# meiqua/6DPose

Measured on AMD Instinct MI355X. Metric: templates*Mpixels matched/sec on 640x480 RGB-D, higher is better.
Workload: dtype u8

## Files before the change

6dpose_amd/csrc/match_bits.hip:

```cpp
#include "match_planes.h"
#include <algorithm>
#include <type_traits>

namespace lm {

static __device__ __forceinline__ uint32_t pack4(uint32_t d) {
    const uint32_t t = ((d | (d >> 1)) & 0x01010101u) | ((d >> 1) & 0x02020202u);
    return (t * 0x01041040u) >> 24;
}
static __device__ __forceinline__ uint32_t pack16(const uint4& v) { return pack4(v.x) | (pack4(v.y) << 8) | (pack4(v.z) << 16) | (pack4(v.w) << 24); }

__global__ void __launch_bounds__(256)
k_pack_bits(BitsBatch B, uint32_t sm_off0, uint32_t records, int NS, int Hd) {
    const uint32_t i = blockIdx.x * 256u + threadIdx.x;
    if (i >= records) return;
    uint4 a, b;
    const size_t at = strip_cells(B.strips[blockIdx.y], sm_off0, i, NS, Hd, a, b);
    uint2 r;
    r.x = pack16(a);
    r.y = pack16(b);
    *reinterpret_cast<uint2*>(B.bits[blockIdx.y] + at) = r;
}

template <int kHi, int kWaves, int kA>
__global__ void __launch_bounds__(256) __attribute__((amdgpu_waves_per_eu(kWaves, kWaves)))
k_local_bits(FrameBatch fb, BitsBatch B, FrameGeom g, const TemplEntry* __restrict__ entries, const uint32_t* __restrict__ feat_word,
             const int32_t* __restrict__ work_pyramids, uint32_t cand_cap, float threshold, uint32_t cap, uint32_t dedupe_cap_slots) {
    constexpr int kN = 4 + kHi;
    constexpr int kS = kN + 3;
    __shared__ unsigned long long s_acc[kMaxBatch][2];
    __shared__ uint32_t s_cnt[kMaxBatch];
    const int lane = threadIdx.x & 63, grp = lane >> 3, j = lane & 7;
    const int nb = fb.nb;
    const LocalShare share = local_share(nb);
    local_prologue(fb, s_cnt, s_acc, cand_cap, dedupe_cap_slots);
    if (B.top_clear_units)
        for (int f = 0; f < nb; ++f)
            for (uint32_t i = blockIdx.x * blockDim.x + threadIdx.x; i < B.top_clear_units; i += gridDim.x * blockDim.x)
                reinterpret_cast<uint4*>(B.top_clear[f])[i] = make_uint4(0u, 0u, 0u, 0u);
    const int src0 = (lane & ~7) << 2;
    const uint32_t rowoff = 16u * (uint32_t)j;
    for (int fr = share.f_lo; fr < share.f_hi; ++fr) {
        const FrameSlot& F = fb.f[fr];
        const BufRsrc bits = make_rsrc(B.bits[fr]);
        const uint32_t nc = s_cnt[fr], ngroups = (nc + 7u) >> 3;
        for (uint32_t gi = share.w_first; gi < ngroups; gi += share.w_step) {
            const uint32_t ci = gi * 8u + (uint32_t)grp;
            const bool valid = ci < nc;
            Candidate cd{0, 0, 0.f, 0};
            if (valid) cd = F.cands[ci];
            const int work = cd.work;
            const int pyr = work_pyramids[work];
            int mx = cd.x, my = cd.y;
            float sim = cd.score;
            bool alive = valid, leave = false;
            uint32_t evals = 0, bytes = 0;
            for (int l = g.levels - 2; l >= 0; --l) {
                const LevelGeom& lv = g.lv[l];
                const TemplEntry e = entries[(size_t)pyr * g.levels + l];
                const LocalWindow win = local_window(lv, e, mx, my, alive, leave);
                const int nfp = win.nfp, nmax = win.nmax;
                const uint32_t* fw = feat_word + e.feat_start;
                uint32_t cA[kN], cB[kN];
#pragma unroll
                for (int k = 0; k < kN; ++k) { cA[k] = 0; cB[k] = 0; }
                uint32_t offx = 0, offy = 0, sx = 0, sy = 0;
                auto batch = [&](int half, uint32_t& eA, uint32_t& eB) {
                    uint4 v[8];
                    uint32_t sh[8];
#pragma unroll
                    for (int u = 0; u < 8; ++u) {
                        const int src = src0 + 4 * (4 * half + (u >> 1));
                        const uint32_t o = (uint32_t)__builtin_amdgcn_ds_bpermute(src, (int)((u & 1) ? offy : offx));
                        sh[u] = (uint32_t)__builtin_amdgcn_ds_bpermute(src, (int)((u & 1) ? sy : sx));
                        v[u] = ld_buf16(bits, o + rowoff, 0u);
                    }
                    uint32_t xa[8], xb[8];
#pragma unroll
                    for (int u = 0; u < 8; ++u) {
                        xa[u] = __builtin_amdgcn_alignbit(v[u].y, v[u].x, sh[u]);
                        xb[u] = __builtin_amdgcn_alignbit(v[u].w, v[u].z, sh[u]);
                    }
                    eA = add8(xa, cA[0], cA[1], cA[2]);
                    eB = add8(xb, cB[0], cB[1], cB[2]);
                };
                uint2 wn = local_fetch(fw, 0, j, nfp);
                for (int f0 = 0; f0 < nmax; f0 += 16) {
                    const uint2 wd = wn;
                    const bool on = f0 + 2 * j < nfp;
                    wn = local_fetch(fw, f0 + 16, j, nfp);
                    local_prep(wd.x, on, win.gxl, win.Kbase, win.HS8, win.zero_off, offx, sx);
                    local_prep(wd.y, on, win.gxl, win.Kbase, win.HS8, win.zero_off, offy, sy);
                    uint32_t e1A, e1B;
                    batch(0, e1A, e1B);
                    if (f0 + 8 < nmax) {
                        uint32_t e2A, e2B;
                        batch(1, e2A, e2B);
                        add_eights2<kN>(cA, e1A, e2A);
                        add_eights2<kN>(cB, e1B, e2B);
                    } else {
                        add_eights1<kN>(cA, e1A);
                        add_eights1<kN>(cB, e1B);
                    }
                }
                uint32_t S[kS];
                {
                    uint32_t n1[kN], n4[kN];
                    local_interleave<kN>(n1, n4, cA, cB);
                    weighted_sum<kA, kN>(S, n1, n4);
                }
                int raw, br, bc;
                local_argmax<kS>(S, j, raw, br, bc);
                local_update(win, lv.T, raw, br, bc, threshold, sim, mx, my, alive, evals, bytes);
            }
            if (valid && j == 0) local_store(F, ci, leave, cap, mx, my, sim, alive, work, s_acc[fr], evals, bytes);
        }
    }
    local_flush_stats(fb, s_acc);
}

void launch_pack_bits(const BitsBatch& B, int nb, const LevelGeom& lv, hipStream_t s) {
    const uint32_t records = (uint32_t)(2 * 8 * lv.T * lv.T) * (uint32_t)lv.NS * (uint32_t)lv.Hd;
    hipLaunchKernelGGL(k_pack_bits, dim3((records + 255) / 256, nb), dim3(256), 0, s, B, lv.sm_off[0], records, lv.NS, lv.Hd);
}
void launch_local_bits(const FrameBatch& fb, const BitsBatch& B, const FrameGeom& g, const BankDev& bank, uint32_t cand_cap, float threshold,
                       uint32_t cap, uint32_t dedupe_cap_slots, int grid_blocks, int max_features, int low_weight, hipStream_t s) {
    with_bits_instance<4, 4>(max_features, low_weight, [&](auto hi, auto waves, auto a) {
        hipLaunchKernelGGL((k_local_bits<hi(), waves(), a()>), dim3(grid_blocks), dim3(256), 0, s, fb, B, g, bank.entries, bank.feat_word, bank.work, cand_cap, threshold, cap,
                           dedupe_cap_slots);
    });
}

__global__ void __launch_bounds__(256)
k_pack_top(TopBits B, uint32_t byte0, uint32_t npairs) {
    const uint32_t i = blockIdx.x * 256u + threadIdx.x;
    if (i >= npairs) return;
    const uint8_t* src = B.lm[blockIdx.y] + byte0 + (size_t)i * 32;
    const uint4 a = *reinterpret_cast<const uint4*>(src), b = *reinterpret_cast<const uint4*>(src + 16);
    *reinterpret_cast<uint2*>(B.bits[blockIdx.y] + (size_t)i * 8) = make_uint2(byte_bits32(a, b, 0) | byte_bits32(a, b, 1), byte_bits32(a, b, 2));
}

template <int kHi, int kWaves, int kA>
__global__ void __launch_bounds__(256) __attribute__((amdgpu_waves_per_eu(kWaves, kWaves)))
k_coarse_bits(FrameBatch fb, TopBits B, LevelGeom lv, int level, int levels, const TemplEntry* __restrict__ entries, const int32_t* __restrict__ feat_off,
              const int32_t* __restrict__ work_pyramids, int num_work, float threshold, uint32_t cap, uint32_t byte0) {
    constexpr int kN = 4 + kHi, kS = kN + 3;
    __shared__ uint32_t s_tot[4];
    __shared__ unsigned long long s_base;
    const FrameSlot& F = fb.f[blockIdx.y];
    const int lane = threadIdx.x & 63;
    const int wave = __builtin_amdgcn_readfirstlane((int)(threadIdx.x >> 6));
    const CoarseHead h = coarse_head((int)blockIdx.x * 4 + wave, num_work, entries, feat_off, work_pyramids, lv, level, levels, threshold);
    const bool live = h.live;
    const int nfp = h.nfp, npos = h.npos, limit = h.limit;
    const int32_t* fo = h.fo;
    const BufRsrc bits = make_rsrc(B.bits[blockIdx.y]);
    for (int P0 = 0; P0 < npos; P0 += 2048) {
        const int pos0 = P0 + 32 * lane;
        uint32_t c1[kN], c4[kN];
#pragma unroll
        for (int k = 0; k < kN; ++k) { c1[k] = 0; c4[k] = 0; }
        if (live && P0 < limit && nfp > 0 && pos0 < limit) {
            auto batch = [&](int f, uint32_t& e1, uint32_t& e4) {
                uint4 v[8];
                uint32_t sh[8];
#pragma unroll
                for (int u = 0; u < 8; ++u) {
                    const uint32_t ob = (uint32_t)fo[f + u] - byte0 + (uint32_t)P0;
                    sh[u] = ob & 31u;
                    v[u] = ld_buf16(bits, (uint32_t)lane * 8u, (ob >> 5) * 8u);
                }
                uint32_t x1[8], x4[8];
#pragma unroll
                for (int u = 0; u < 8; ++u) {
                    x1[u] = __builtin_amdgcn_alignbit(v[u].z, v[u].x, sh[u]);
                    x4[u] = __builtin_amdgcn_alignbit(v[u].w, v[u].y, sh[u]);
                }
                e1 = add8(x1, c1[0], c1[1], c1[2]);
                e4 = add8(x4, c4[0], c4[1], c4[2]);
            };
            for (int f = 0; f < nfp; f += 16) {
                uint32_t a1, a4;
                batch(f, a1, a4);
                if (f + 8 < nfp) {
                    uint32_t b1, b4;
                    batch(f + 8, b1, b4);
                    add_eights2<kN>(c1, a1, b1);
                    add_eights2<kN>(c4, a4, b4);
                } else {
                    add_eights1<kN>(c1, a1);
                    add_eights1<kN>(c4, a4);
                }
            }
        }
        uint32_t S[kS];
        weighted_sum<kA, kN>(S, c1, c4);
        uint32_t summed;
        uint32_t hit_mask = coarse_hit_mask<kS>(S, h.rmin, h.zero_passes, limit, npos, pos0, summed);
        if (!live) hit_mask = 0;
// ... 132 lines not shown
```

6dpose_amd/csrc/match_parts.hip:

```cpp
#include "match_planes.h"

namespace lm {

template <int kHi, int kWaves, int kA>
__global__ void __launch_bounds__(256) __attribute__((amdgpu_waves_per_eu(kWaves, kWaves)))
k_coarse_parts(FrameBatch fb, TopBits B, LevelGeom lv, int level, int levels, const TemplEntry* __restrict__ entries, const PartEntry* __restrict__ parts,
               const int32_t* __restrict__ part_off, const int32_t* __restrict__ work_pyramids, int num_work, float threshold, int min_parts, uint32_t cap, uint32_t byte0) {
    constexpr int kN = 4 + kHi, kS = kN + 3;
    __shared__ uint32_t s_tot[4];
    __shared__ unsigned long long s_base;
    const FrameSlot& F = fb.f[blockIdx.y];
    const int lane = threadIdx.x & 63;
    const int wave = __builtin_amdgcn_readfirstlane((int)(threadIdx.x >> 6));
    const CoarseHead h = coarse_head((int)blockIdx.x * 4 + wave, num_work, entries, part_off, work_pyramids, lv, level, levels, threshold);
    const bool live = h.live;
    const int npos = h.npos, limit = h.limit;
    const PartEntry* pe = parts + (size_t)work_pyramids[h.work] * levels + level;
    const BufRsrc bits = make_rsrc(B.bits[blockIdx.y]);
    for (int P0 = 0; P0 < npos; P0 += 2048) {
        const int pos0 = P0 + 32 * lane;
        const bool loads = live && P0 < limit && pos0 < limit;
        uint32_t S[kS];
#pragma unroll
        for (int k = 0; k < kS; ++k) S[k] = 0;
        uint32_t q0 = 0, q1 = 0, q2 = 0, summed = 0;
#pragma unroll 1
        for (int p = 0; p < 4; ++p) {
            const int np = pe->n[p], npp = pe->npad[p];
            const int32_t* fo = part_off + pe->start[p];
            uint32_t c1[kN], c4[kN];
#pragma unroll
            for (int k = 0; k < kN; ++k) { c1[k] = 0; c4[k] = 0; }
            if (loads) {
                auto batch = [&](int f, uint32_t& e1, uint32_t& e4) {
                    uint4 v[8];
                    uint32_t sh[8];
#pragma unroll
                    for (int u = 0; u < 8; ++u) {
                        const uint32_t ob = (uint32_t)fo[f + u] - byte0 + (uint32_t)P0;
                        sh[u] = ob & 31u;
                        v[u] = ld_buf16(bits, (uint32_t)lane * 8u, (ob >> 5) * 8u);
                    }
                    uint32_t x1[8], x4[8];
#pragma unroll
                    for (int u = 0; u < 8; ++u) {
                        x1[u] = __builtin_amdgcn_alignbit(v[u].z, v[u].x, sh[u]);
                        x4[u] = __builtin_amdgcn_alignbit(v[u].w, v[u].y, sh[u]);
                    }
                    e1 = add8(x1, c1[0], c1[1], c1[2]);
                    e4 = add8(x4, c4[0], c4[1], c4[2]);
                };
                for (int f = 0; f < npp; f += 16) {
                    uint32_t a1, a4;
                    batch(f, a1, a4);
                    if (f + 8 < npp) {
                        uint32_t b1, b4;
                        batch(f + 8, b1, b4);
                        add_eights2<kN>(c1, a1, b1);
                        add_eights2<kN>(c4, a4, b4);
                    } else {
                        add_eights1<kN>(c1, a1);
                        add_eights1<kN>(c4, a4);
                    }
                }
            }
            uint32_t Sp[kS];
            weighted_sum<kA, kN>(Sp, c1, c4);
            const int rmin = (pe->eligible >> p) & 1u ? coarse_rmin(threshold, np) : (1 << kS);
            count3_add(q0, q1, q2, coarse_hit_mask<kS>(Sp, rmin, false, limit, npos, pos0, summed));
            sliced_add<kS>(S, Sp);
        }
        uint32_t hit_mask = count3_ge(q0, q1, q2, min_parts);
        if (!live) hit_mask = 0;
        int total;
        const unsigned long long slot = coarse_reserve_slots(s_tot, s_base, F.counters, hit_mask, lane, wave, total);
        if (total > 0)
            coarse_emit<kS>(hit_mask, summed, S, slot, cap, pos0, h.Wd, h.T, h.offset, h.nf, h.work, F.cands);
    }
}

template <int kHi, int kWaves, int kA>
__global__ void __launch_bounds__(256) __attribute__((amdgpu_waves_per_eu(kWaves, kWaves)))
k_local_parts(FrameBatch fb, BitsBatch B, FrameGeom g, const TemplEntry* __restrict__ entries, const PartEntry* __restrict__ parts, const uint32_t* __restrict__ part_word,
              const int32_t* __restrict__ work_pyramids, uint32_t cand_cap, float threshold, int min_parts, uint32_t cap, uint32_t dedupe_cap_slots) {
    constexpr int kN = 4 + kHi;
    constexpr int kS = kN + 3;
    __shared__ unsigned long long s_acc[kMaxBatch][2];
    __shared__ uint32_t s_cnt[kMaxBatch];
    const int lane = threadIdx.x & 63, grp = lane >> 3, j = lane & 7;
    const int nb = fb.nb;
    const LocalShare share = local_share(nb);
    local_prologue(fb, s_cnt, s_acc, cand_cap, dedupe_cap_slots);
    if (B.top_clear_units)
        for (int f = 0; f < nb; ++f)
            for (uint32_t i = blockIdx.x * blockDim.x + threadIdx.x; i < B.top_clear_units; i += gridDim.x * blockDim.x)
                reinterpret_cast<uint4*>(B.top_clear[f])[i] = make_uint4(0u, 0u, 0u, 0u);
    const int src0 = (lane & ~7) << 2;
    const uint32_t rowoff = 16u * (uint32_t)j;
    for (int fr = share.f_lo; fr < share.f_hi; ++fr) {
        const FrameSlot& F = fb.f[fr];
        const BufRsrc bits = make_rsrc(B.bits[fr]);
        const uint32_t nc = s_cnt[fr], ngroups = (nc + 7u) >> 3;
        for (uint32_t gi = share.w_first; gi < ngroups; gi += share.w_step) {
            const uint32_t ci = gi * 8u + (uint32_t)grp;
            const bool valid = ci < nc;
            Candidate cd{0, 0, 0.f, 0};
            if (valid) cd = F.cands[ci];
            const int work = cd.work;
            const int pyr = work_pyramids[work];
            int mx = cd.x, my = cd.y;
            float sim = cd.score;
            bool alive = valid, leave = false;
            uint32_t evals = 0, bytes = 0;
            for (int l = g.levels - 2; l >= 0; --l) {
                const LevelGeom& lv = g.lv[l];
                const TemplEntry e = entries[(size_t)pyr * g.levels + l];
                const uint32_t ei = (uint32_t)(pyr * g.levels + l);
                const LocalWindow win = local_window(lv, e, mx, my, alive, leave);
                const int my_bound = (parts[ei].eligible >> (j & 3)) & 1u ? local_rmin(threshold, (int)parts[ei].n[j & 3]) : (1 << kS);
                uint32_t S[kS];
#pragma unroll
                for (int k = 0; k < kS; ++k) S[k] = 0;
                uint32_t q0 = 0, q1 = 0, q2 = 0;
#pragma unroll 1
                for (int p = 0; p < 4; ++p) {
                    const int nfp = win.run ? (int)parts[ei].npad[p] : 0;
                    int nmax = nfp;
#pragma unroll
                    for (int o = 32; o > 0; o >>= 1) { const int t = __shfl_xor(nmax, o, 64); nmax = t > nmax ? t : nmax; }
                    nmax = __builtin_amdgcn_readfirstlane(nmax);
                    const uint32_t* fw = part_word + parts[ei].start[p];
                    uint32_t cA[kN], cB[kN];
#pragma unroll
                    for (int k = 0; k < kN; ++k) { cA[k] = 0; cB[k] = 0; }
                    uint32_t offx = 0, offy = 0, sx = 0, sy = 0;
                    auto batch = [&](int half, uint32_t& eA, uint32_t& eB) {
                        uint4 v[8];
                        uint32_t sh[8];
#pragma unroll
                        for (int u = 0; u < 8; ++u) {
                            const int src = src0 + 4 * (4 * half + (u >> 1));
                            const uint32_t o = (uint32_t)__builtin_amdgcn_ds_bpermute(src, (int)((u & 1) ? offy : offx));
                            sh[u] = (uint32_t)__builtin_amdgcn_ds_bpermute(src, (int)((u & 1) ? sy : sx));
                            v[u] = ld_buf16(bits, o + rowoff, 0u);
                        }
                        uint32_t xa[8], xb[8];
#pragma unroll
                        for (int u = 0; u < 8; ++u) {
                            xa[u] = __builtin_amdgcn_alignbit(v[u].y, v[u].x, sh[u]);
                            xb[u] = __builtin_amdgcn_alignbit(v[u].w, v[u].z, sh[u]);
                        }
                        eA = add8(xa, cA[0], cA[1], cA[2]);
                        eB = add8(xb, cB[0], cB[1], cB[2]);
                    };
                    uint2 wn = local_fetch(fw, 0, j, nfp);
                    for (int f0 = 0; f0 < nmax; f0 += 16) {
                        const uint2 wd = wn;
                        const bool on = f0 + 2 * j < nfp;
                        wn = local_fetch(fw, f0 + 16, j, nfp);
                        local_prep(wd.x, on, win.gxl, win.Kbase, win.HS8, win.zero_off, offx, sx);
                        local_prep(wd.y, on, win.gxl, win.Kbase, win.HS8, win.zero_off, offy, sy);
                        uint32_t e1A, e1B;
                        batch(0, e1A, e1B);
                        if (f0 + 8 < nmax) {
                            uint32_t e2A, e2B;
                            batch(1, e2A, e2B);
                            add_eights2<kN>(cA, e1A, e2A);
                            add_eights2<kN>(cB, e1B, e2B);
                        } else {
                            add_eights1<kN>(cA, e1A);
                            add_eights1<kN>(cB, e1B);
                        }
                    }
                    uint32_t Sp[kS];
                    {
                        uint32_t n1[kN], n4[kN];
                        local_interleave<kN>(n1, n4, cA, cB);
                        weighted_sum<kA, kN>(Sp, n1, n4);
                    }
                    const int bound = __shfl(my_bound, (lane & ~7) + p, 64);
                    count3_add(q0, q1, q2, sliced_ge<kS>(Sp, bound));
                    sliced_add<kS>(S, Sp);
                }
                int raw, br, bc;
                local_argmax<kS>(S, j, raw, br, bc);
                const int at = raw > 0 ? 2 * bc + (br & 1) : 0;
                const int mine = (int)((q0 >> at) & 1u) + 2 * (int)((q1 >> at) & 1u) + 4 * (int)((q2 >> at) & 1u);
                const int passed = __shfl(mine, (lane & ~7) + (raw > 0 ? br >> 1 : 0), 64);
                local_update(win, lv.T, raw, br, bc, -__builtin_inff() , sim, mx, my, alive, evals, bytes);
                if (win.run && passed < min_parts) alive = false;
            }
            if (valid && j == 0) local_store(F, ci, leave, cap, mx, my, sim, alive, work, s_acc[fr], evals, bytes);
        }
    }
    local_flush_stats(fb, s_acc);
}

void launch_coarse_parts(const FrameBatch& fb, const TopBits& B, const FrameGeom& g, const BankDev& bank, const PartsDev& parts, int num_work, float threshold, uint32_t cap,
                         uint32_t byte0, int max_features, int low_weight, hipStream_t s) {
    if (num_work <= 0 || fb.nb <= 0) return;
    const int level = g.levels - 1;
    with_bits_instance<5, 4>(max_features, low_weight, [&](auto hi, auto waves, auto a) {
        hipLaunchKernelGGL((k_coarse_parts<hi(), waves(), a()>), dim3((num_work + 3) / 4, fb.nb), dim3(256), 0, s, fb, B, g.lv[level], level, g.levels, bank.entries, parts.table,
                           parts.feat_off, bank.work, num_work, threshold, parts.min_parts, cap, byte0);
    });
}
void launch_local_parts(const FrameBatch& fb, const BitsBatch& B, const FrameGeom& g, const BankDev& bank, const PartsDev& parts, uint32_t cand_cap, float threshold,
                        uint32_t cap, uint32_t dedupe_cap_slots, int grid_blocks, int max_features, int low_weight, hipStream_t s) {
    with_bits_instance<4, 3>(max_features, low_weight, [&](auto hi, auto waves, auto a) {
        hipLaunchKernelGGL((k_local_parts<hi(), waves(), a()>), dim3(grid_blocks), dim3(256), 0, s, fb, B, g, bank.entries, parts.table, parts.feat_word, bank.work, cand_cap, threshold,
                           parts.min_parts, cap, dedupe_cap_slots);
    });
}

}
```

6dpose_amd/csrc/match_planes.h:

```cpp
#pragma once
#include "match_device.h"
#include <type_traits>

namespace lm {


static __device__ __forceinline__ int coarse_rmin(float threshold, int nf) {
    int rmin = (int)(threshold * (float)(4 * nf) / 100.f);
    if (!(rmin >= 0)) rmin = 0;
    if (rmin > 4 * nf + 1) rmin = 4 * nf + 1;
    while (rmin > 0 && score_of(rmin, nf) > threshold) --rmin;
    while (rmin <= 4 * nf && !(score_of(rmin, nf) > threshold)) ++rmin;
    return rmin;
}

static __device__ __forceinline__ int local_rmin(float threshold, int nf) {
    int rmin = (int)(threshold * (float)(4 * nf) / 100.f);
    if (!(rmin >= 0)) rmin = 0;
    if (rmin > 4 * nf + 1) rmin = 4 * nf + 1;
    while (rmin > 0 && score_of(rmin - 1, nf) >= threshold) --rmin;
    while (rmin <= 4 * nf && !(score_of(rmin, nf) >= threshold)) ++rmin;
    return rmin;
}

struct CoarseHead {
    bool live;
    int work, nf, nfp;
    const int32_t* fo;
    int Wd, T, npos;
    int limit;
    int offset;
    int rmin;
    bool zero_passes;
};
static __device__ __forceinline__ CoarseHead coarse_head(int work_raw, int num_work, const TemplEntry* __restrict__ entries, const int32_t* __restrict__ feat_off,
                                                         const int32_t* __restrict__ work_pyramids, const LevelGeom& lv, int level, int levels, float threshold) {
    CoarseHead h;
    h.live = work_raw < num_work;
    h.work = h.live ? work_raw : num_work - 1;
    const int pyr = work_pyramids[h.work];
    const TemplEntry e = entries[(size_t)pyr * levels + level];
    h.nf = e.nf; h.nfp = e.nf_padded;
    h.fo = feat_off + e.feat_start;
    const int Hd = lv.Hd;
    h.Wd = lv.Wd; h.T = lv.T; h.npos = h.Wd * Hd;
    const int wf = (e.width - 1) / h.T + 1, hf = (e.height - 1) / h.T + 1;
    const int tp = (Hd - hf) * h.Wd + (h.Wd - wf) + 1;
    h.offset = h.T / 2 + (h.T % 2 - 1);
    h.limit = tp < h.npos ? tp : h.npos;
    h.rmin = coarse_rmin(threshold, h.nf);
    h.zero_passes = score_of(0, h.nf) > threshold;
    return h;
}

template <int kS>
static __device__ __forceinline__ uint32_t coarse_hit_mask(const uint32_t (&S)[kS], int rmin, bool zero_passes, int limit, int npos, int pos0, uint32_t& summed) {
    uint32_t gt = 0, eq = 0xFFFFFFFFu;
#pragma unroll
    for (int k = kS - 1; k >= 0; --k) {
        if ((rmin >> k) & 1) eq &= S[k];
        else { gt |= eq & S[k]; eq &= ~S[k]; }
    }
    const uint32_t hit_mask = rmin < (1 << kS) ? (gt | eq) : 0u;
    const int sums = limit - pos0;
    summed = sums >= 32 ? 0xFFFFFFFFu : (sums > 0 ? (1u << sums) - 1u : 0u);
    const int inmap = npos - pos0;
    const uint32_t mapped = inmap >= 32 ? 0xFFFFFFFFu : (inmap > 0 ? (1u << inmap) - 1u : 0u);
    return (hit_mask & summed) | (zero_passes ? (mapped & ~summed) : 0u);
}

static __device__ __forceinline__ unsigned long long coarse_reserve_slots(uint32_t (&s_tot)[4], unsigned long long& s_base, unsigned long long* __restrict__ counters,
                                                                          uint32_t hit_mask, int lane, int wave, int& total) {
    const int before = wave_excl_scan(__popc(hit_mask), lane, total);
    if (lane == 0) s_tot[wave] = (uint32_t)total;
    __syncthreads();
    if (threadIdx.x == 0) {
        const unsigned long long all = (unsigned long long)s_tot[0] + s_tot[1] + s_tot[2] + s_tot[3];
        s_base = all ? atomicAdd(&counters[0], all) : 0ull;
    }
    __syncthreads();
    unsigned long long slot = s_base + (unsigned long long)before;
    for (int w = 0; w < wave; ++w) slot += s_tot[w];
    __syncthreads();
    return slot;
}

template <int kS>
static __device__ __forceinline__ void coarse_emit(uint32_t hit_mask, uint32_t summed, const uint32_t (&S)[kS], unsigned long long slot, uint32_t cap, int pos0,
                                                   int Wd, int T, int offset, int nf, int work, Candidate* __restrict__ cands) {
    uint32_t m = hit_mask;
    while (m) {
        const int b = __ffs((int)m) - 1;
        m &= m - 1;
        if (slot < cap) {
            int raw = 0;
            if ((summed >> b) & 1u) {
#pragma unroll
                for (int k = 0; k < kS; ++k) raw |= (int)((S[k] >> b) & 1u) << k;
            }
            const int jpos = pos0 + b;
            const int cy = jpos / Wd, cx = jpos - cy * Wd;
            Candidate c;
            c.x = cx * T + offset; c.y = cy * T + offset; c.score = score_of(raw, nf); c.work = work;
            cands[slot] = c;
        }
        ++slot;
    }
}


struct LocalShare { int f_lo, f_hi; uint32_t w_first, w_step; };
static __device__ __forceinline__ LocalShare local_share(int nb) {
    LocalShare s;
    s.f_lo = 0; s.f_hi = nb;
    s.w_first = blockIdx.x * (blockDim.x >> 6) + (threadIdx.x >> 6); s.w_step = gridDim.x * (blockDim.x >> 6);
    if (nb > 1 && nb <= 8 && (gridDim.x & 7) == 0) {
        const int xcd = (int)(blockIdx.x & 7);
        s.f_lo = xcd % nb; s.f_hi = s.f_lo + 1;
        const uint32_t mine = (uint32_t)((7 - s.f_lo) / nb + 1);
        const uint32_t wpb = blockDim.x >> 6;
        s.w_first = ((blockIdx.x >> 3) * mine + (uint32_t)(xcd / nb)) * wpb + (threadIdx.x >> 6);
        s.w_step = (gridDim.x >> 3) * mine * wpb;
    }
    return s;
}

static __device__ __forceinline__ void local_prologue(const FrameBatch& fb, uint32_t (&s_cnt)[kMaxBatch], unsigned long long (&s_acc)[kMaxBatch][2], uint32_t cand_cap,
                                                      uint32_t dedupe_cap_slots) {
    const int nb = fb.nb;
    if ((int)threadIdx.x < nb) {
        const unsigned long long nc = fb.f[threadIdx.x].counters[0] & kCandMask;
        s_cnt[threadIdx.x] = nc < cand_cap ? (uint32_t)nc : cand_cap;
        s_acc[threadIdx.x][0] = 0; s_acc[threadIdx.x][1] = 0;
    }
    __syncthreads();
    for (int f = 0; f < nb; ++f) {
        unsigned long long* table = fb.f[f].dedupe_table;
        if (!table) continue;
        const uint32_t tsize = dedupe_slots_for(s_cnt[f], dedupe_cap_slots);
        for (uint32_t i = blockIdx.x * blockDim.x + threadIdx.x; i < tsize; i += gridDim.x * blockDim.x) table[i] = ~0ull;
    }
}

struct LocalWindow {
    int x, y;
    int gx, gy;
    bool all_in;
    bool run;
    int nf, nfp;
    int nmax;
    uint32_t Kbase, gxl;
    uint32_t zero_off, HS8;
};
static __device__ __forceinline__ LocalWindow local_window(const LevelGeom& lv, const TemplEntry& e, int mx, int my, bool alive, bool& leave) {
    LocalWindow w;
    const int T = lv.T, W = lv.W, H = lv.H, Wd = lv.Wd, Hd = lv.Hd;
    const int border = 8 * T;
    w.HS8 = (uint32_t)Hd * 8u;
    w.zero_off = (lv.sm_off[1] + 8u * (uint32_t)(T * T) * ((uint32_t)lv.NS * (uint32_t)Hd * 16u)) >> 1;
    const int max_x = W - e.width - border, max_y = H - e.height - border;
    int x = mx * 2 + 1, y = my * 2 + 1;
    x = x > border ? x : border;  y = y > border ? y : border;
    x = x < max_x ? x : max_x;    y = y < max_y ? y : max_y;
    w.x = x; w.y = y;
    w.gx = x / T - 8; w.gy = y / T - 8;
    const int off_x = w.gx * T, off_y = w.gy * T;
    w.all_in = e.min_x >= 0 && e.min_y >= 0 && w.gx >= 0 && w.gy >= 0 &&
               ((e.max_x + off_x) / T + 16 <= Wd) && ((e.max_y + off_y) / T + 16 <= Hd);
    const bool want = alive && !leave;
    leave = leave || (want && !w.all_in);
    w.run = want && w.all_in;
    w.nf = e.nf; w.nfp = w.run ? (int)e.nf_padded : 0;
    int nmax = w.nfp;
#pragma unroll
    for (int o = 32; o > 0; o >>= 1) { const int t = __shfl_xor(nmax, o, 64); nmax = t > nmax ? t : nmax; }
    w.nmax = __builtin_amdgcn_readfirstlane(nmax);
    w.Kbase = (uint32_t)(((w.gx >> 4) * Hd + w.gy) * 8);
    w.gxl = (uint32_t)(w.gx & 15);
    return w;
}

static __device__ __forceinline__ uint2 local_fetch(const uint32_t* fw, int f0, int j, int nfp) {
    uint2 w = make_uint2(0u, 0u);
    if (f0 + 2 * j < nfp) w = *reinterpret_cast<const uint2*>(fw + f0 + 2 * j);
    return w;
}
static __device__ __forceinline__ void local_prep(uint32_t w, bool on, uint32_t gxl, uint32_t Kbase, uint32_t HS8, uint32_t zero_off, uint32_t& off, uint32_t& s2) {
    s2 = ((w & 15u) + gxl) << 1;
    const uint32_t o = ((w & ~15u) >> 1) + Kbase + ((s2 >> 5) ? HS8 : 0u);
    off = on ? o : zero_off;
}

template <int kN>
static __device__ __forceinline__ void local_interleave(uint32_t (&n1)[kN], uint32_t (&n4)[kN], const uint32_t (&cA)[kN], const uint32_t (&cB)[kN]) {
#pragma unroll
    for (int k = 0; k < kN; ++k) {
        n1[k] = (cA[k] & 0x55555555u) | ((cB[k] << 1) & 0xAAAAAAAAu);
        n4[k] = ((cA[k] >> 1) & 0x55555555u) | (cB[k] & 0xAAAAAAAAu);
    }
}

template <int kS>
static __device__ __forceinline__ void local_argmax(const uint32_t (&S)[kS], int j, int& raw, int& br, int& bc) {
    uint32_t mask = 0xFFFFFFFFu, val = 0;
#pragma unroll
    for (int k = kS - 1; k >= 0; --k) {
        const uint32_t t = mask & S[k];
        if (t) { mask = t; val |= 1u << k; }
    }
    const uint32_t upper = mask & 0x55555555u;
    const uint32_t pick = upper ? upper : mask;
    const uint32_t bitp = (uint32_t)__ffs((int)pick) - 1u;
    const uint32_t pos = ((2u * (uint32_t)j + (bitp & 1u)) << 4) + (bitp >> 1);
    uint32_t key = (val << 8) | (255u - pos);
#pragma unroll
    for (int o = 1; o < 8; o <<= 1) { const uint32_t t = (uint32_t)__shfl_xor((int)key, o, 64); key = t > key ? t : key; }
    raw = (int)(key >> 8);
    br = -1; bc = -1;
    if (raw > 0) {
        const int idx = 255 - (int)(key & 0xFF);
        br = idx >> 4; bc = idx & 15;
    }
}

static __device__ __forceinline__ void local_update(const LocalWindow& w, int T, int raw, int br, int bc, float threshold, float& sim, int& mx, int& my, bool& alive,
                                                    uint32_t& evals, uint32_t& bytes) {
    const float best = raw > 0 ? score_of(raw, w.nf) : 0.f;
    if (w.run) {
        const int offset = T / 2 + (T % 2 - 1);
        ++evals;
        bytes += 256u * (uint32_t)w.nf;
        sim = best;
        mx = (w.x / T - 8 + bc) * T + offset;
        my = (w.y / T - 8 + br) * T + offset;
        if (sim < threshold) alive = false;
    }
}

static __device__ __forceinline__ void local_store(const FrameSlot& F, uint32_t ci, bool leave, uint32_t cap, int mx, int my, float sim, bool alive, int work,
                                                   unsigned long long (&acc)[2], uint32_t evals, uint32_t bytes) {
    F.todo[ci] = leave ? 1 : 0;
    if (!leave) {
        if (ci < cap) {
            Candidate m;
            m.x = mx; m.y = my; m.score = sim;
            m.work = alive ? work : -1;
            F.matches_dev[ci] = m;
        }
        atomicAdd(&acc[0], (unsigned long long)evals);
        atomicAdd(&acc[1], (unsigned long long)bytes);
    }
}
static __device__ __forceinline__ void local_flush_stats(const FrameBatch& fb, unsigned long long (&s_acc)[kMaxBatch][2]) {
    __syncthreads();
    if ((int)threadIdx.x < fb.nb && s_acc[threadIdx.x][0] != 0) {
        unsigned long long* st = fb.f[threadIdx.x].counters + 8 + 2 * (blockIdx.x & (kStatShards - 1));
        atomicAdd(st, s_acc[threadIdx.x][0]);
        atomicAdd(st + 1, s_acc[threadIdx.x][1]);
    }
}


static __device__ __forceinline__ uint32_t byte_bits16(const uint4& v, int sh) {
    auto four = [](uint32_t d, int sh) -> uint32_t { return ((((d >> sh) & 0x01010101u) * 0x01020408u) >> 24) & 0xFu; };
    return four(v.x, sh) | (four(v.y, sh) << 4) | (four(v.z, sh) << 8) | (four(v.w, sh) << 12);
}
static __device__ __forceinline__ uint32_t byte_bits32(const uint4& a, const uint4& b, int sh) { return byte_bits16(a, sh) | (byte_bits16(b, sh) << 16); }

static __device__ __forceinline__ size_t strip_cells(const uint8_t* strips, uint32_t sm_off0, uint32_t i, int NS, int Hd, uint4& a, uint4& b) {
    const uint32_t q = i / (uint32_t)Hd, s = q % (uint32_t)NS;
    const uint8_t* src = strips + sm_off0 + (size_t)i * 16;
    a = *reinterpret_cast<const uint4*>(src);
    b = make_uint4(0, 0, 0, 0);
    if (s + 1 < (uint32_t)NS) b = *reinterpret_cast<const uint4*>(src + (size_t)Hd * 16);
    return (sm_off0 >> 1) + (size_t)i * 8;
}

// ... 14 lines not shown
```

6dpose_amd/csrc/match_wide.hip:

```cpp
#include "match_planes.h"

namespace lm {

template <int kN>
static __device__ __forceinline__ void weighted_sum_wide(uint32_t (&S)[kN + 3], const uint32_t (&n1)[kN], const uint32_t (&n2)[kN], const uint32_t (&n4)[kN]) {
    constexpr int kS = kN + 3;
    uint32_t t[kN + 2];
    uint32_t carry = 0;
    t[0] = n1[0];
#pragma unroll
    for (int k = 1; k < kN + 2; ++k) csa(t[k], carry, k < kN ? n1[k] : 0u, k - 1 < kN ? n2[k - 1] : 0u, carry);
    carry = 0;
    S[0] = t[0]; S[1] = t[1];
#pragma unroll
    for (int k = 2; k < kS; ++k) csa(S[k], carry, k < kN + 2 ? t[k] : 0u, k - 2 < kN ? n4[k - 2] : 0u, carry);
}

static __device__ __forceinline__ uint32_t wide4_set0(uint32_t d) { return ((((d & 0x01010101u) | ((d >> 1) & 0x02020202u)) * 0x01041040u) >> 24); }
static __device__ __forceinline__ uint32_t wide4_set1(uint32_t d) { return ((((d >> 1) & 0x01010101u) * 0x01041040u) >> 24); }
static __device__ __forceinline__ uint32_t wide16_set0(const uint4& v) { return wide4_set0(v.x) | (wide4_set0(v.y) << 8) | (wide4_set0(v.z) << 16) | (wide4_set0(v.w) << 24); }
static __device__ __forceinline__ uint32_t wide16_set1(const uint4& v) { return wide4_set1(v.x) | (wide4_set1(v.y) << 8) | (wide4_set1(v.z) << 16) | (wide4_set1(v.w) << 24); }

__global__ void __launch_bounds__(256)
k_pack_wide(BitsBatch B, WidePlanes P, uint32_t sm_off0, uint32_t records, int NS, int Hd) {
    const uint32_t i = blockIdx.x * 256u + threadIdx.x;
    if (i >= records) return;
    uint4 a, b;
    const size_t at = strip_cells(B.strips[blockIdx.y], sm_off0, i, NS, Hd, a, b);
    *reinterpret_cast<uint2*>(B.bits[blockIdx.y] + at) = make_uint2(wide16_set0(a), wide16_set0(b));
    *reinterpret_cast<uint2*>(P.set1[blockIdx.y] + at) = make_uint2(wide16_set1(a), wide16_set1(b));
}

template <int kHi, int kWaves, int kInFlight>
__global__ void __launch_bounds__(256) __attribute__((amdgpu_waves_per_eu(kWaves, kWaves)))
k_local_wide(FrameBatch fb, BitsBatch B, WidePlanes P, FrameGeom g, const TemplEntry* __restrict__ entries, const uint32_t* __restrict__ feat_word,
             const int32_t* __restrict__ work_pyramids, uint32_t cand_cap, float threshold, uint32_t cap, uint32_t dedupe_cap_slots) {
    constexpr int kN = 4 + kHi;
    constexpr int kS = kN + 3;
    __shared__ unsigned long long s_acc[kMaxBatch][2];
    __shared__ uint32_t s_cnt[kMaxBatch];
    const int lane = threadIdx.x & 63, grp = lane >> 3, j = lane & 7;
    const LocalShare share = local_share(fb.nb);
    local_prologue(fb, s_cnt, s_acc, cand_cap, dedupe_cap_slots);
    const int src0 = (lane & ~7) << 2;
    const uint32_t rowoff = 16u * (uint32_t)j;
    for (int fr = share.f_lo; fr < share.f_hi; ++fr) {
        const FrameSlot& F = fb.f[fr];
        const BufRsrc bits0 = make_rsrc(B.bits[fr]), bits1 = make_rsrc(P.set1[fr]);
        const uint32_t nc = s_cnt[fr], ngroups = (nc + 7u) >> 3;
        for (uint32_t gi = share.w_first; gi < ngroups; gi += share.w_step) {
            const uint32_t ci = gi * 8u + (uint32_t)grp;
            const bool valid = ci < nc;
            Candidate cd{0, 0, 0.f, 0};
            if (valid) cd = F.cands[ci];
            const int work = cd.work;
            const int pyr = work_pyramids[work];
            int mx = cd.x, my = cd.y;
            float sim = cd.score;
            bool alive = valid, leave = false;
            uint32_t evals = 0, bytes = 0;
            for (int l = g.levels - 2; l >= 0; --l) {
                const LevelGeom& lv = g.lv[l];
                const TemplEntry e = entries[(size_t)pyr * g.levels + l];
                const LocalWindow win = local_window(lv, e, mx, my, alive, leave);
                const int nfp = win.nfp, nmax = win.nmax;
                const uint32_t* fw = feat_word + e.feat_start;
                uint32_t cA[kN], cB[kN], cC[kN];
#pragma unroll
                for (int k = 0; k < kN; ++k) { cA[k] = 0; cB[k] = 0; cC[k] = 0; }
                uint32_t offx = 0, offy = 0, sx = 0, sy = 0;
                auto batch = [&](int half, uint32_t& eA, uint32_t& eB, uint32_t& eC) {
                    uint32_t xa[8], xb[8], xc[8];
#pragma unroll
                    for (int q = 0; q < 8; q += kInFlight) {
                        uint4 v[kInFlight], w[kInFlight];
                        uint32_t sh[kInFlight];
#pragma unroll
                        for (int u = 0; u < kInFlight; ++u) {
                            const int src = src0 + 4 * (4 * half + ((q + u) >> 1));
                            const uint32_t o = (uint32_t)__builtin_amdgcn_ds_bpermute(src, (int)(((q + u) & 1) ? offy : offx));
                            sh[u] = (uint32_t)__builtin_amdgcn_ds_bpermute(src, (int)(((q + u) & 1) ? sy : sx));
                            v[u] = ld_buf16(bits0, o + rowoff, 0u);
                            w[u] = ld_buf16(bits1, o + rowoff, 0u);
                        }
#pragma unroll
                        for (int u = 0; u < kInFlight; ++u) {
                            xa[q + u] = __builtin_amdgcn_alignbit(v[u].y, v[u].x, sh[u]);
                            xb[q + u] = __builtin_amdgcn_alignbit(v[u].w, v[u].z, sh[u]);
                            xc[q + u] = __builtin_amdgcn_alignbit(w[u].y, w[u].x, sh[u]) | (__builtin_amdgcn_alignbit(w[u].w, w[u].z, sh[u]) << 1);
                        }
                    }
                    eA = add8(xa, cA[0], cA[1], cA[2]);
                    eB = add8(xb, cB[0], cB[1], cB[2]);
                    eC = add8(xc, cC[0], cC[1], cC[2]);
                };
                uint2 wn = local_fetch(fw, 0, j, nfp);
                for (int f0 = 0; f0 < nmax; f0 += 16) {
                    const uint2 wd = wn;
                    const bool on = f0 + 2 * j < nfp;
                    wn = local_fetch(fw, f0 + 16, j, nfp);
                    local_prep(wd.x, on, win.gxl, win.Kbase, win.HS8, win.zero_off, offx, sx);
                    local_prep(wd.y, on, win.gxl, win.Kbase, win.HS8, win.zero_off, offy, sy);
                    uint32_t e1A, e1B, e1C;
                    batch(0, e1A, e1B, e1C);
                    if (f0 + 8 < nmax) {
                        uint32_t e2A, e2B, e2C;
                        batch(1, e2A, e2B, e2C);
                        add_eights2<kN>(cA, e1A, e2A);
                        add_eights2<kN>(cB, e1B, e2B);
                        add_eights2<kN>(cC, e1C, e2C);
                    } else {
                        add_eights1<kN>(cA, e1A);
                        add_eights1<kN>(cB, e1B);
                        add_eights1<kN>(cC, e1C);
                    }
                }
                uint32_t S[kS];
                {
                    uint32_t n1[kN], n4[kN];
                    local_interleave<kN>(n1, n4, cA, cB);
                    weighted_sum_wide<kN>(S, n1, cC, n4);
                }
                int raw, br, bc;
                local_argmax<kS>(S, j, raw, br, bc);
                local_update(win, lv.T, raw, br, bc, threshold, sim, mx, my, alive, evals, bytes);
            }
            if (valid && j == 0) local_store(F, ci, leave, cap, mx, my, sim, alive, work, s_acc[fr], evals, bytes);
        }
    }
    local_flush_stats(fb, s_acc);
}

void launch_pack_wide(const BitsBatch& B, const WidePlanes& P, int nb, const LevelGeom& lv, hipStream_t s) {
    const uint32_t records = (uint32_t)(2 * 8 * lv.T * lv.T) * (uint32_t)lv.NS * (uint32_t)lv.Hd;
    hipLaunchKernelGGL(k_pack_wide, dim3((records + 255) / 256, nb), dim3(256), 0, s, B, P, lv.sm_off[0], records, lv.NS, lv.Hd);
}
void launch_local_wide(const FrameBatch& fb, const BitsBatch& B, const WidePlanes& P, const FrameGeom& g, const BankDev& bank, uint32_t cand_cap, float threshold,
                       uint32_t cap, uint32_t dedupe_cap_slots, int grid_blocks, int max_features, hipStream_t s) {
#define LM_LAUNCH_LOCAL_WIDE(HI, WAVES, FLY) \
    hipLaunchKernelGGL((k_local_wide<HI, WAVES, FLY>), dim3(grid_blocks), dim3(256), 0, s, fb, B, P, g, bank.entries, bank.feat_word, bank.work, cand_cap, threshold, cap, dedupe_cap_slots)
    if (max_features > kBitsSmallMax) LM_LAUNCH_LOCAL_WIDE(10, 3, 4); else LM_LAUNCH_LOCAL_WIDE(5, 4, 2);
#undef LM_LAUNCH_LOCAL_WIDE
}

__global__ void __launch_bounds__(256)
k_pack_top_wide(TopBits B, WidePlanes P, uint32_t byte0, uint32_t npairs) {
    const uint32_t i = blockIdx.x * 256u + threadIdx.x;
    if (i >= npairs) return;
    const uint8_t* src = B.lm[blockIdx.y] + byte0 + (size_t)i * 32;
    const uint4 a = *reinterpret_cast<const uint4*>(src), b = *reinterpret_cast<const uint4*>(src + 16);
    *reinterpret_cast<uint2*>(B.bits[blockIdx.y] + (size_t)i * 8) = make_uint2(byte_bits32(a, b, 0), byte_bits32(a, b, 2));
    *reinterpret_cast<uint2*>(P.set1[blockIdx.y] + (size_t)i * 8) = make_uint2(byte_bits32(a, b, 1), 0u);
}

template <int kHi, int kWaves, int kInFlight>
__global__ void __launch_bounds__(256) __attribute__((amdgpu_waves_per_eu(kWaves, kWaves)))
k_coarse_wide(FrameBatch fb, TopBits B, WidePlanes P, LevelGeom lv, int level, int levels, const TemplEntry* __restrict__ entries, const int32_t* __restrict__ feat_off,
              const int32_t* __restrict__ work_pyramids, int num_work, float threshold, uint32_t cap, uint32_t byte0) {
    constexpr int kN = 4 + kHi, kS = kN + 3;
    __shared__ uint32_t s_tot[4];
    __shared__ unsigned long long s_base;
    const FrameSlot& F = fb.f[blockIdx.y];
    const int lane = threadIdx.x & 63;
    const int wave = __builtin_amdgcn_readfirstlane((int)(threadIdx.x >> 6));
    const CoarseHead h = coarse_head((int)blockIdx.x * 4 + wave, num_work, entries, feat_off, work_pyramids, lv, level, levels, threshold);
    const bool live = h.live;
    const int nfp = h.nfp, npos = h.npos, limit = h.limit;
    const int32_t* fo = h.fo;
    const BufRsrc bits0 = make_rsrc(B.bits[blockIdx.y]), bits1 = make_rsrc(P.set1[blockIdx.y]);
    for (int P0 = 0; P0 < npos; P0 += 2048) {
        const int pos0 = P0 + 32 * lane;
        uint32_t c1[kN], c2[kN], c4[kN];
#pragma unroll
        for (int k = 0; k < kN; ++k) { c1[k] = 0; c2[k] = 0; c4[k] = 0; }
        if (live && P0 < limit && nfp > 0 && pos0 < limit) {
            auto batch = [&](int f, uint32_t& e1, uint32_t& e2, uint32_t& e4) {
                uint32_t x1[8], x2[8], x4[8];
#pragma unroll
                for (int q = 0; q < 8; q += kInFlight) {
                    uint4 v[kInFlight], w[kInFlight];
                    uint32_t sh[kInFlight];
#pragma unroll
                    for (int u = 0; u < kInFlight; ++u) {
                        const uint32_t ob = (uint32_t)fo[f + q + u] - byte0 + (uint32_t)P0;
                        sh[u] = ob & 31u;
                        v[u] = ld_buf16(bits0, (uint32_t)lane * 8u, (ob >> 5) * 8u);
                        w[u] = ld_buf16(bits1, (uint32_t)lane * 8u, (ob >> 5) * 8u);
                    }
#pragma unroll
                    for (int u = 0; u < kInFlight; ++u) {
                        x1[q + u] = __builtin_amdgcn_alignbit(v[u].z, v[u].x, sh[u]);
                        x4[q + u] = __builtin_amdgcn_alignbit(v[u].w, v[u].y, sh[u]);
                        x2[q + u] = __builtin_amdgcn_alignbit(w[u].z, w[u].x, sh[u]);
                    }
                }
                e1 = add8(x1, c1[0], c1[1], c1[2]);
                e2 = add8(x2, c2[0], c2[1], c2[2]);
                e4 = add8(x4, c4[0], c4[1], c4[2]);
            };
            for (int f = 0; f < nfp; f += 16) {
                uint32_t a1, a2, a4;
                batch(f, a1, a2, a4);
                if (f + 8 < nfp) {
// ... 40 lines not shown
```

Baseline: 10.61 million.

## Deal refinement candidate groups across waves by global count, balanced per XCD

The refinement kernels now split work by counting all candidate groups across every frame in the batch. Each XCD gets a contiguous slice of that global range, and waves stride within the slice. Before, whole frames were pinned to XCDs by frame index, regardless of how many candidates each frame had. The change aims to remove the load imbalance that occurs when frames have unequal candidate counts or the batch size does not divide 8. In exchange, each wave does some extra scalar work computing the split after the prologue, and an XCD may now touch data from several frames.

```diff
diff --git a/6dpose_amd/csrc/local_deal.h b/6dpose_amd/csrc/local_deal.h
--- /dev/null
+++ b/6dpose_amd/csrc/local_deal.h
@@ -0,0 +1,56 @@
+#pragma once
+#include <stdint.h>
+
+#if defined(__HIPCC__) || defined(__CUDACC__)
+#define LM_DEAL_HD __host__ __device__ __forceinline__
+#else
+#define LM_DEAL_HD inline
+#endif
+
+namespace lm {
+
+struct LocalShare {
+    int f_lo, f_hi;
+    uint32_t lo, hi;
+    uint32_t w, w_step;
+    uint32_t base;
+    LM_DEAL_HD bool segment(uint32_t at, uint32_t n, uint32_t& first, uint32_t& end) const {
+        const uint32_t a = at > lo ? at : lo, b = at + n < hi ? at + n : hi;
+        first = 0; end = 0;
+        if (a >= b) return false;
+        uint32_t t = lo + w;
+        if (t < a) t += (a - t + w_step - 1) / w_step * w_step;
+        if (t >= b) return false;
+        first = t - at; end = b - at;
+        return true;
+    }
+};
+
+LM_DEAL_HD LocalShare local_share(int nb, const uint32_t* count, uint32_t grid, uint32_t block, uint32_t wpb, uint32_t wave) {
+    uint32_t G = 0;
+    for (int f = 0; f < nb; ++f) G += (count[f] + 7u) >> 3;
+    LocalShare s;
+    if ((grid & 7u) == 0) {
+        const uint32_t xcd = block & 7u;
+        s.lo = (uint32_t)((uint64_t)xcd * G >> 3);
+        s.hi = (uint32_t)((uint64_t)(xcd + 1u) * G >> 3);
+        s.w = (block >> 3) * wpb + wave;
+        s.w_step = (grid >> 3) * wpb;
+    } else {
+        s.lo = 0; s.hi = G;
+        s.w = block * wpb + wave;
+        s.w_step = grid * wpb;
+    }
+    s.f_lo = 0; s.f_hi = 0; s.base = 0;
+    uint32_t at = 0;
+    for (int f = 0; f < nb; ++f) {
+        const uint32_t n = (count[f] + 7u) >> 3;
+        if (at + n <= s.lo && s.lo < s.hi) { s.f_lo = f + 1; s.base = at + n; }
+        if (at < s.hi && n > 0 && s.lo < s.hi) s.f_hi = f + 1;
+        at += n;
+    }
+    if (s.f_hi < s.f_lo) s.f_hi = s.f_lo;
+    return s;
+}
+
+}
diff --git a/6dpose_amd/csrc/match_bits.hip b/6dpose_amd/csrc/match_bits.hip
--- a/6dpose_amd/csrc/match_bits.hip
+++ b/6dpose_amd/csrc/match_bits.hip
@@ -32,19 +32,21 @@
     __shared__ uint32_t s_cnt[kMaxBatch];
     const int lane = threadIdx.x & 63, grp = lane >> 3, j = lane & 7;
     const int nb = fb.nb;
-    const LocalShare share = local_share(nb);
     local_prologue(fb, s_cnt, s_acc, cand_cap, dedupe_cap_slots);
+    const LocalShare share = local_share_of_wave(nb, s_cnt);
     if (B.top_clear_units)
         for (int f = 0; f < nb; ++f)
             for (uint32_t i = blockIdx.x * blockDim.x + threadIdx.x; i < B.top_clear_units; i += gridDim.x * blockDim.x)
                 reinterpret_cast<uint4*>(B.top_clear[f])[i] = make_uint4(0u, 0u, 0u, 0u);
     const int src0 = (lane & ~7) << 2;
     const uint32_t rowoff = 16u * (uint32_t)j;
+    uint32_t at = share.base;
     for (int fr = share.f_lo; fr < share.f_hi; ++fr) {
         const FrameSlot& F = fb.f[fr];
         const BufRsrc bits = make_rsrc(B.bits[fr]);
-        const uint32_t nc = s_cnt[fr], ngroups = (nc + 7u) >> 3;
-        for (uint32_t gi = share.w_first; gi < ngroups; gi += share.w_step) {
+        uint32_t nc, g_first, g_end;
+        local_frame_groups(share, s_cnt, fr, at, nc, g_first, g_end);
+        for (uint32_t gi = g_first; gi < g_end; gi += share.w_step) {
             const uint32_t ci = gi * 8u + (uint32_t)grp;
             const bool valid = ci < nc;
             Candidate cd{0, 0, 0.f, 0};
diff --git a/6dpose_amd/csrc/match_parts.hip b/6dpose_amd/csrc/match_parts.hip
--- a/6dpose_amd/csrc/match_parts.hip
+++ b/6dpose_amd/csrc/match_parts.hip
@@ -89,19 +89,21 @@
     __shared__ uint32_t s_cnt[kMaxBatch];
     const int lane = threadIdx.x & 63, grp = lane >> 3, j = lane & 7;
     const int nb = fb.nb;
-    const LocalShare share = local_share(nb);
     local_prologue(fb, s_cnt, s_acc, cand_cap, dedupe_cap_slots);
+    const LocalShare share = local_share_of_wave(nb, s_cnt);
     if (B.top_clear_units)
         for (int f = 0; f < nb; ++f)
             for (uint32_t i = blockIdx.x * blockDim.x + threadIdx.x; i < B.top_clear_units; i += gridDim.x * blockDim.x)
                 reinterpret_cast<uint4*>(B.top_clear[f])[i] = make_uint4(0u, 0u, 0u, 0u);
     const int src0 = (lane & ~7) << 2;
     const uint32_t rowoff = 16u * (uint32_t)j;
+    uint32_t at = share.base;
     for (int fr = share.f_lo; fr < share.f_hi; ++fr) {
         const FrameSlot& F = fb.f[fr];
         const BufRsrc bits = make_rsrc(B.bits[fr]);
-        const uint32_t nc = s_cnt[fr], ngroups = (nc + 7u) >> 3;
-        for (uint32_t gi = share.w_first; gi < ngroups; gi += share.w_step) {
+        uint32_t nc, g_first, g_end;
+        local_frame_groups(share, s_cnt, fr, at, nc, g_first, g_end);
+        for (uint32_t gi = g_first; gi < g_end; gi += share.w_step) {
             const uint32_t ci = gi * 8u + (uint32_t)grp;
             const bool valid = ci < nc;
             Candidate cd{0, 0, 0.f, 0};
diff --git a/6dpose_amd/csrc/match_planes.h b/6dpose_amd/csrc/match_planes.h
--- a/6dpose_amd/csrc/match_planes.h
+++ b/6dpose_amd/csrc/match_planes.h
@@ -1,5 +1,6 @@
 #pragma once
 #include "match_device.h"
+#include "local_deal.h"
 #include <type_traits>
 
 namespace lm {
@@ -109,20 +110,23 @@
 }
 
 
-struct LocalShare { int f_lo, f_hi; uint32_t w_first, w_step; };
-static __device__ __forceinline__ LocalShare local_share(int nb) {
+static __device__ __forceinline__ LocalShare local_share_of_wave(int nb, const uint32_t (&s_cnt)[kMaxBatch]) {
+    const LocalShare v = local_share(nb, s_cnt, gridDim.x, blockIdx.x, blockDim.x >> 6, threadIdx.x >> 6);
     LocalShare s;
-    s.f_lo = 0; s.f_hi = nb;
-    s.w_first = blockIdx.x * (blockDim.x >> 6) + (threadIdx.x >> 6); s.w_step = gridDim.x * (blockDim.x >> 6);
-    if (nb > 1 && nb <= 8 && (gridDim.x & 7) == 0) {
-        const int xcd = (int)(blockIdx.x & 7);
-        s.f_lo = xcd % nb; s.f_hi = s.f_lo + 1;
-        const uint32_t mine = (uint32_t)((7 - s.f_lo) / nb + 1);
-        const uint32_t wpb = blockDim.x >> 6;
-        s.w_first = ((blockIdx.x >> 3) * mine + (uint32_t)(xcd / nb)) * wpb + (threadIdx.x >> 6);
-        s.w_step = (gridDim.x >> 3) * mine * wpb;
-    }
+    s.f_lo = __builtin_amdgcn_readfirstlane(v.f_lo); s.f_hi = __builtin_amdgcn_readfirstlane(v.f_hi);
+    s.lo = (uint32_t)__builtin_amdgcn_readfirstlane((int)v.lo); s.hi = (uint32_t)__builtin_amdgcn_readfirstlane((int)v.hi);
+    s.w = (uint32_t)__builtin_amdgcn_readfirstlane((int)v.w); s.w_step = (uint32_t)__builtin_amdgcn_readfirstlane((int)v.w_step);
+    s.base = (uint32_t)__builtin_amdgcn_readfirstlane((int)v.base);
     return s;
+}
+static __device__ __forceinline__ void local_frame_groups(const LocalShare& share, const uint32_t (&s_cnt)[kMaxBatch], int fr, uint32_t& at, uint32_t& nc,
+                                                          uint32_t& first, uint32_t& end) {
+    nc = (uint32_t)__builtin_amdgcn_readfirstlane((int)s_cnt[fr]);
+    const uint32_t n = (nc + 7u) >> 3;
+    uint32_t a, b;
+    share.segment(at, n, a, b);
+    at += n;
+    first = (uint32_t)__builtin_amdgcn_readfirstlane((int)a); end = (uint32_t)__builtin_amdgcn_readfirstlane((int)b);
 }
 
 static __device__ __forceinline__ void local_prologue(const FrameBatch& fb, uint32_t (&s_cnt)[kMaxBatch], unsigned long long (&s_acc)[kMaxBatch][2], uint32_t cand_cap,
diff --git a/6dpose_amd/csrc/match_wide.hip b/6dpose_amd/csrc/match_wide.hip
--- a/6dpose_amd/csrc/match_wide.hip
+++ b/6dpose_amd/csrc/match_wide.hip
@@ -40,15 +40,17 @@
     __shared__ unsigned long long s_acc[kMaxBatch][2];
     __shared__ uint32_t s_cnt[kMaxBatch];
     const int lane = threadIdx.x & 63, grp = lane >> 3, j = lane & 7;
-    const LocalShare share = local_share(fb.nb);
     local_prologue(fb, s_cnt, s_acc, cand_cap, dedupe_cap_slots);
+    const LocalShare share = local_share_of_wave(fb.nb, s_cnt);
     const int src0 = (lane & ~7) << 2;
     const uint32_t rowoff = 16u * (uint32_t)j;
+    uint32_t at = share.base;
     for (int fr = share.f_lo; fr < share.f_hi; ++fr) {
         const FrameSlot& F = fb.f[fr];
         const BufRsrc bits0 = make_rsrc(B.bits[fr]), bits1 = make_rsrc(P.set1[fr]);
-        const uint32_t nc = s_cnt[fr], ngroups = (nc + 7u) >> 3;
-        for (uint32_t gi = share.w_first; gi < ngroups; gi += share.w_step) {
+        uint32_t nc, g_first, g_end;
+        local_frame_groups(share, s_cnt, fr, at, nc, g_first, g_end);
+        for (uint32_t gi = g_first; gi < g_end; gi += share.w_step) {
             const uint32_t ci = gi * 8u + (uint32_t)grp;
             const bool valid = ci < nc;
             Candidate cd{0, 0, 0.f, 0};
diff --git a/profiles/local_balance.py b/profiles/local_balance.py
--- /dev/null
+++ b/profiles/local_balance.py
@@ -0,0 +1,75 @@
+import argparse
+import json
+import os
+import statistics
+import sys
+
+ROOT = os.path.dirname(os.path.dirname(os.path.abspath(__file__)))
+ap = argparse.ArgumentParser()
+ap.add_argument("--label", default="new")
+ap.add_argument("--lib", default=None, help="another build of libamdlinemod.so (default: the tree's)")
+ap.add_argument("--launches", type=int, default=9)
+ap.add_argument("--templates", type=int, default=2000)
+ap.add_argument("--equal", action="store_true", help="every frame of a launch is the same frame: equal candidate counts (8 frames: the rule gives XCD f frame f exactly)")
+ap.add_argument("--table", nargs="+", metavar="JSONL", help="print the table of these result files instead of measuring")
+args = ap.parse_args()
+
+if args.table:
+    rows = {}
+    for path in args.table:
+        for line in open(path):
+            if line.startswith("{"):
+                r = json.loads(line)
+                rows.setdefault((r["label"], r["nb"]), []).extend(r["local_us"])
+    labels = sorted({k[0] for k in rows}, key=lambda s: (s != "parent", s))
+    print("refinement (local_ms of the launch), microseconds: median [min, max] (launches)")
+    print("%-4s" % "nb" + "".join("%-34s" % l for l in labels))
+    for nb in range(1, 9):
+        cells = []
+        for l in labels:
+            v = rows.get((l, nb), [])
+            cells.append("%-34s" % ("%.1f [%.1f, %.1f] (%d)" % (statistics.median(v), min(v), max(v), len(v)) if v else "-"))
+        print("%-4d" % nb + "".join(cells))
+    sys.exit(0)
+
+if args.lib:
+    os.environ["AMD_LINEMOD_LIB"] = os.path.abspath(args.lib)
+for p in (os.path.join(ROOT, "tests"), os.path.join(ROOT, "oracle"), os.path.join(ROOT, "6dpose_amd")):
+    sys.path.insert(0, p)
+import numpy as np
+import linemodLevelup_pybind as lm
+import synth
+
+W, H, T, NFEAT, THR = 640, 480, [4, 8], (150, 75), 75.0
+rgb0, dep0 = synth.make_frame(0, W, H)
+frames = [(rgb0, dep0)]
+for k in range(1, 16):
+    rng = np.random.default_rng(1000 + k)
+    rgb = np.clip(rgb0.astype(np.int16) + rng.integers(-2, 3, rgb0.shape), 0, 255).astype(np.uint8)
+    dn = dep0.astype(np.int32) + rng.integers(-1, 2, dep0.shape)
+    frames.append((np.ascontiguousarray(rgb), np.where(dep0 > 0, np.clip(dn, 300, 65535), 0).astype(np.uint16)))
+det = lm.Detector(NFEAT[0], T, device=0)
+det.addClassPacked("_probe", np.zeros((0, 3), np.int32), np.zeros(1, np.int32), np.zeros((0, 2), np.int32))
+det.setFrame(list(frames[0]))
+det.matchResident(THR, ["_probe"])
+quant = [(det.readStage(l, 0).reshape(H >> l, W >> l), det.readStage(l, 1).reshape(H >> l, W >> l)) for l in range(2)]
+det.addClassPacked("obj00", *synth.make_planted_bank(1234, args.templates, quant, T, NFEAT))
+det.setBatchQueue(0)
+at = 0
+for nb in range(1, 9):
+    det.setBatch(nb)
+    us, cands = [], []
+    for rep in range(3 + args.launches):
+        for b in range(nb):
+            det.submitFrame(list(frames[(at + (0 if args.equal else b)) % len(frames)]), THR, ["obj00"])
+        at += nb
+        for b in range(nb):
+            det.collect(sort_unique=False, distinct=True)
+            tm = det.lastTimings()
+            assert tm["batch_frames"] == nb, tm
+            if rep >= 3:
+                cands.append(tm["coarse_candidates"])
+                if b == 0:
+                    us.append(1e3 * tm["local_ms"])
+    print(json.dumps({"label": args.label, "nb": nb, "local_us": [round(v, 2) for v in us], "candidates_per_frame_mean": sum(cands) / len(cands),
+                      "paths": det.getPaths()}), flush=True)
```

After: 10.55 million. About the same (-0.5%).
